# instadeepai/FrameDiPT

Measured on AMD Instinct MI355X. Metric: residue*diffusion-steps/sec, higher is better.
Workload: dtype fp16

## Files before the change

framedipt_amd/csrc/frames.hip:

```cpp
#include "common.hpp"
#include "kernels.hpp"
#include "philox.hpp"

#pragma clang fp contract(off)

__device__ __forceinline__ void d_quat_to_rot(const float* q, float* R) {
  const float a = q[0], b = q[1], c = q[2], d = q[3];
  R[0] = a * a + b * b - c * c - d * d; R[1] = 2 * b * c - 2 * a * d; R[2] = 2 * b * d + 2 * a * c;
  R[3] = 2 * b * c + 2 * a * d; R[4] = a * a - b * b + c * c - d * d; R[5] = 2 * c * d - 2 * a * b;
  R[6] = 2 * b * d - 2 * a * c; R[7] = 2 * c * d + 2 * a * b; R[8] = a * a - b * b - c * c + d * d;
}
__device__ __forceinline__ void d_quat_mul(const float* p, const float* q, float* o) {
  o[0] = p[0] * q[0] - p[1] * q[1] - p[2] * q[2] - p[3] * q[3];
  o[1] = p[0] * q[1] + p[1] * q[0] + p[2] * q[3] - p[3] * q[2];
  o[2] = p[0] * q[2] - p[1] * q[3] + p[2] * q[0] + p[3] * q[1];
  o[3] = p[0] * q[3] + p[1] * q[2] - p[2] * q[1] + p[3] * q[0];
}
__device__ __forceinline__ void d_quat_mul_vec(const float* q, const float* v, float* o) {
  o[0] = -q[1] * v[0] - q[2] * v[1] - q[3] * v[2];
  o[1] = q[0] * v[0] + q[2] * v[2] - q[3] * v[1];
  o[2] = q[0] * v[1] - q[1] * v[2] + q[3] * v[0];
  o[3] = q[0] * v[2] + q[1] * v[1] - q[2] * v[0];
}
__device__ __forceinline__ void d_invert_quat(const float* q, float* o) {
// ... 573 lines not shown
int fd_split_rigids(long n, const float* t7, float cs, const float* res_mask, const float* fixed_mask, float* quat,
                    float* trans, float* dmask, FdStep step, hipStream_t st) {
  hipLaunchKernelGGL(split_rigids_kernel, dim3(cdiv(n, 256)), dim3(256), 0, st, n, t7, cs, res_mask, fixed_mask, quat, trans, dmask, step);
  FD_CHECK_LAUNCH();
  return FDIPT_OK;
}

__global__ void finish_kernel(long n, const float* __restrict__ quat, const float* __restrict__ trans, float cs,
                              const float* __restrict__ psi_un, int ld_psi, const float* __restrict__ gt_psi,
                              const float* __restrict__ fixed_mask, float* __restrict__ rigids,
                              float* __restrict__ psi) {
  const long r = (long)blockIdx.x * blockDim.x + threadIdx.x;
  if (r >= n) return;
  for (int c = 0; c < 4; ++c) rigids[r * 7 + c] = quat[r * 4 + c];
  for (int c = 0; c < 3; ++c) fd_st(rigids + r * 7 + 4 + c, trans[r * 3 + c] / cs);
  const float a = psi_un[r * ld_psi], bq = psi_un[r * ld_psi + 1];
  const float den = sqrtf(fmaxf(a * a + bq * bq, 1e-8f));
  const float dm = 1.f - fixed_mask[r];
  psi[r * 2] = dm * (a / den) + (1.f - dm) * gt_psi[r * 2];
  psi[r * 2 + 1] = dm * (bq / den) + (1.f - dm) * gt_psi[r * 2 + 1];
}
int fd_finish(long n, const float* quat, const float* trans, float cs, const float* psi_un, int ld_psi,
              const float* gt_psi, const float* fixed_mask, float* rigids, float* psi, hipStream_t st) {
  hipLaunchKernelGGL(finish_kernel, dim3(cdiv(n, 256)), dim3(256), 0, st, n, quat, trans, cs, psi_un, ld_psi, gt_psi,
                     fixed_mask, rigids, psi);
  FD_CHECK_LAUNCH();
  return FDIPT_OK;
}

struct FeatsExtra {
  const float *t7, *res_mask; float cs; float *quat, *trans, *dmask;
  const float *w1i, *w1j, *b1; int cz; float *pi, *pj;
  FdStep step;
};
template <bool KEPT>
__global__ void build_feats_kernel(int B, int N, int use_aatype, int E, const int32_t* __restrict__ aatype,
                                   const float* __restrict__ t_emb_, const float* __restrict__ t_emb_eps,
                                   const float* __restrict__ fixed_mask, const float* __restrict__ idx_emb,
                                   float* __restrict__ node_feat, int ld_node, float* __restrict__ pte, int ld_pte,
                                   FeatsExtra x) {
  __shared__ float pte_s[128];
  const FdStepRows at = fd_step_rows<KEPT>(x.step);
  const float* __restrict__ t_emb = t_emb_ + at.step * B * E;
  if (x.t7) x.t7 += at.state_in * B * N * 7;
  const long r = blockIdx.x;
  const int b = (int)(r / N);
  const float fm = fixed_mask[r];
  const int d1 = E + 1 + (use_aatype ? 21 : 0);
  if (x.t7 && threadIdx.x < 8) {
    const int c = threadIdx.x;
    if (c < 4) x.quat[r * 4 + c] = x.t7[r * 7 + c];
    else if (c < 7) x.trans[r * 3 + c - 4] = x.t7[r * 7 + c] * x.cs;
    else x.dmask[r] = (1.f - fm) * x.res_mask[r];
  }
  for (int c = threadIdx.x; c < ld_node; c += blockDim.x) {
    float v = 0.f;
    int cc = c;
    if (use_aatype) {
      if (c < 21) { v = (aatype[r] == c) ? 1.f : 0.f; cc = -1; } else cc = c - 21;
    }
    if (cc >= 0) {
      if (cc < E) v = (use_aatype && fm != 0.f) ? t_emb_eps[cc] : t_emb[b * E + cc];
      else if (cc == E) v = fm;
      else if (cc < 2 * E + 1) v = idx_emb[r * E + (cc - E - 1)];
    }
    node_feat[r * ld_node + c] = v;
    if (c < ld_pte) {
      pte[r * ld_pte + c] = c < d1 ? v : 0.f;
      if (x.pi && c < 128) pte_s[c] = c < d1 ? v : 0.f;
    }
  }
  if (!x.pi) return;
  __syncthreads();
  for (int c = threadIdx.x; c < x.cz; c += blockDim.x) {
    const float4* wi = (const float4*)(x.w1i + (long)c * ld_pte);
    const float4* wj = (const float4*)(x.w1j + (long)c * ld_pte);
    float si = 0.f, sj = 0.f;
    for (int k = 0; k < ld_pte / 4; ++k) {
      const float4 a = wi[k], bq = wj[k];
      const float p0 = pte_s[4 * k], p1 = pte_s[4 * k + 1], p2 = pte_s[4 * k + 2], p3 = pte_s[4 * k + 3];
      si = fmaf(p3, a.w, fmaf(p2, a.z, fmaf(p1, a.y, fmaf(p0, a.x, si))));
      sj = fmaf(p3, bq.w, fmaf(p2, bq.z, fmaf(p1, bq.y, fmaf(p0, bq.x, sj))));
    }
    x.pi[r * x.cz + c] = si + x.b1[c];
    x.pj[r * x.cz + c] = sj;
  }
}
int fd_build_feats(int B, int N, int use_aatype, int E, const int32_t* aatype, const float* t_emb, const float* t_emb_eps,
                   const float* fixed_mask, const float* idx_emb, float* node_feat, int ld_node, float* pte, int ld_pte,
                   const float* t7, const float* res_mask, float cs, float* quat, float* trans, float* dmask, const float* w1i,
                   const float* w1j, const float* b1, int cz, float* pi, float* pj, FdStep step, hipStream_t st) {
  if (use_aatype && (!aatype || !t_emb_eps)) return FDIPT_EINVAL;
  if (pi && (ld_pte > 128 || (ld_pte & 3))) return FDIPT_EINVAL;
  FeatsExtra x = {t7, res_mask, cs, quat, trans, dmask, w1i, w1j, b1, cz, pi, pj, step};
  const auto kernel = step.kept() ? build_feats_kernel<true> : build_feats_kernel<false>;
  hipLaunchKernelGGL(kernel, dim3(B * N), dim3(128), 0, st, B, N, use_aatype, E, aatype, t_emb, t_emb_eps,
                     fixed_mask, idx_emb, node_feat, ld_node, pte, ld_pte, x);
  FD_CHECK_LAUNCH();
  return FDIPT_OK;
}

int fd_rot_score(int B, int N, const float* qt, int ld_t, const float* q0, int ld_0, const double* sigma,
                 const float* res_mask, double* score, hipStream_t st) {
  ScoreTail x = {};
  hipLaunchKernelGGL(rot_score_kernel<false>, dim3(cdiv((long)B * N, FD_THREADS / RS_LANES)), dim3(FD_THREADS), 0, st, B, N, qt, ld_t, q0,
                     ld_0, sigma, res_mask, score, x);
  FD_CHECK_LAUNCH();
  return FDIPT_OK;
}
int fd_score_tail(int B, int N, const float* rigids_t, const float* quat, const float* trans, float cs, const float* psi_un,
                  int ld_psi, const float* gt_psi, const float* fixed_mask, const float* res_mask, const double* sigma,
                  const float* t, float min_b, float max_b, float* rigids, float* psi, double* rot_score, float* trans_score,
                  float* ca_out, const float* hid, int ld_hid, int c_hid, const float* torf_w, const float* torf_b,
                  const double* score_table, const double* omega_edges, int n_omega, const int32_t* aatype, const void* bb_tables,
                  float* atom37, float* atom14, FdStep step, hipStream_t st) {
  if (hid && ((c_hid & 3) || (ld_hid & 3))) return FDIPT_EINVAL;
  if (score_table && (!omega_edges || n_omega < 2)) return FDIPT_EINVAL;
  if ((atom37 || atom14) && !bb_tables) return FDIPT_EINVAL;
  ScoreTail x = {trans, cs, psi_un, ld_psi, gt_psi, fixed_mask, t, min_b, max_b, rigids, psi, trans_score, ca_out,
                 hid, torf_w, torf_b, ld_hid, c_hid, score_table, omega_edges, n_omega, aatype, (const BackboneTables*)bb_tables, atom37, atom14,
                 step};
  const auto kernel = step.kept() ? rot_score_kernel<true> : rot_score_kernel<false>;
  hipLaunchKernelGGL(kernel, dim3(cdiv((long)B * N, FD_THREADS / RS_LANES)), dim3(FD_THREADS), 0, st, B, N, rigids_t, 7,
                     quat, 4, sigma, res_mask, rot_score, x);
  FD_CHECK_LAUNCH();
  return FDIPT_OK;
}
int fd_trans_score(int B, int N, const float* tt, int ld_t, const float* t0, int ld_0, const float* t, float min_b,
                   float max_b, float cs, const float* res_mask, float* score, hipStream_t st) {
// ... 592 lines not shown
```

framedipt_amd/csrc/kernels.hpp:

```cpp
#pragma once
#include <hip/hip_runtime.h>
#include <stdint.h>

typedef unsigned short half_t;

struct EdgeTransArgs {
  int B, N;
  const void* z_in;
  void* z_out;
  const float* e;
  const void *w1, *w2, *wf;
  const float *b1, *b2, *bf, *gamma, *beta;
  const float* res_mask;
  float* trace;
  unsigned long long* clock = nullptr;
};

struct EdgeEmbedArgs {
  int B, N, n_rel, rel_off, num_bins;
  const float* pi;
  const float* pj;
  const float* rtab;
  const float* dtab;
  const float* edges;
// ... 301 lines not shown
                 const float* beta, const float* rowmask, float* out, int ldo, hipStream_t st);
int fd_f32_to_half(long n, const float* in, half_t* out, hipStream_t st);
int fd_edge_transition(int precision, int cz, int cb, const EdgeTransArgs& a, hipStream_t st);
int fd_edge_embed(int precision, int cz, const EdgeEmbedArgs& a, hipStream_t st);
int fd_attention(int precision, int ipa, const AttnArgs& a, hipStream_t st);
int fd_ipa_attention_f32_supported(const AttnArgs& a);
int fd_ipa_attention_f32(const AttnArgs& a, hipStream_t st);
int fd_opair(int precision, const OPairArgs& a, hipStream_t st, int long_keys = 0);
int fd_opair_mfma_eligible(int precision, const OPairArgs& a, int long_keys = 0);
int fd_opair_pz(const OPairArgs& a, hipStream_t st);
int fd_pair_bias2(int B, int N, int H, const void* z, const void* wb, const float* bb, float* out, int frag, hipStream_t st);
int fd_pair_bias_f32(long n_pairs, int H, int CZ, const float* z, const float* wb, const float* bb, float* out, hipStream_t st);
int fd_points(const PointsArgs& a, hipStream_t st);
int fd_compose_q_update(long n, float* quat, float* trans, const float* upd, int ld_upd, const float* mask, hipStream_t st);
struct FdStep {
  const int32_t* cursor = nullptr;
  const int32_t* frame_rows = nullptr;
  int ring = 0;
  bool valid() const { return (ring & ~1) == 0 && (cursor || (!frame_rows && !ring)); }
  bool kept() const { return frame_rows != nullptr || ring != 0; }
};
struct FdStepRows { long step, state_in, state_out, frame; };
template <bool KEPT = true>
__device__ __forceinline__ FdStepRows fd_step_rows(const FdStep& s) {
  if (!s.cursor) return {0, 0, 0, 0};
  const long k = s.cursor[0];
  if (!KEPT) return {k, k, k + 1, k};
  return {k, s.ring ? (k & 1) : k, s.ring ? ((k + 1) & 1) : k + 1, s.frame_rows ? (long)s.frame_rows[k] : k};
}
int fd_split_rigids(long n, const float* t7, float cs, const float* res_mask, const float* fixed_mask, float* quat,
                    float* trans, float* dmask, FdStep step, hipStream_t st);
int fd_finish(long n, const float* quat, const float* trans, float cs, const float* psi_un, int ld_psi,
              const float* gt_psi, const float* fixed_mask, float* rigids, float* psi, hipStream_t st);
int fd_build_feats(int B, int N, int use_aatype, int E, const int32_t* aatype, const float* t_emb, const float* t_emb_eps,
                   const float* fixed_mask, const float* idx_emb, float* node_feat, int ld_node, float* pte, int ld_pte,
                   const float* t7, const float* res_mask, float cs, float* quat, float* trans, float* dmask, const float* w1i,
                   const float* w1j, const float* b1, int cz, float* pi, float* pj, FdStep step, hipStream_t st);
int fd_score_tail(int B, int N, const float* rigids_t, const float* quat, const float* trans, float cs, const float* psi_un,
                  int ld_psi, const float* gt_psi, const float* fixed_mask, const float* res_mask, const double* sigma,
                  const float* t, float min_b, float max_b, float* rigids, float* psi, double* rot_score, float* trans_score,
                  float* ca_out, const float* hid, int ld_hid, int c_hid, const float* torf_w, const float* torf_b,
                  const double* score_table, const double* omega_edges, int n_omega, const int32_t* aatype, const void* bb_tables,
                  float* atom37, float* atom14, FdStep step, hipStream_t st);
int fd_rot_score(int B, int N, const float* qt, int ld_t, const float* q0, int ld_0, const double* sigma,
                 const float* res_mask, double* score, hipStream_t st);
int fd_trans_score(int B, int N, const float* tt, int ld_t, const float* t0, int ld_0, const float* t, float min_b,
                   float max_b, float cs, const float* res_mask, float* score, hipStream_t st);
int fd_backbone(int n, const float* t7, const float* rot, const float* trans, int ld_trans, const float* psi,
                const int32_t* aatype, const void* tables, float* atom37, float* atom14, hipStream_t st,
                FdStep step = {});
```

framedipt_amd/csrc/model.hip:

```cpp
#include <math.h>
#include <string.h>

#include <vector>

#include "common.hpp"
#include "kernels.hpp"

struct LinW { long w, b; int out, in; };
struct LNW { long g, b; int d; };
#define FD_MAX_BLOCKS 8
#define FD_MAX_TL 4
struct TfLayer { LinW inp, outp, l1, l2; LNW n1, n2; };
struct BlockW {
  long head_w;
  LinW q, kv, qp, kvp, lb, dz, out, rbf;
  LNW ipa_ln;
  LinW skip;
  TfLayer tf[FD_MAX_TL];
  LinW post, t1, t2, t3;
  LNW tln;
  LinW bb;
  LinW et_init, et1, et2, etf;
  LNW et_ln;
};
// ... 560 lines not shown
}

enum { OP_ALL, OP_EMBED, OP_POINTS, OP_IPA, OP_ET };
struct OpSel {
  int kind = OP_ALL, block = 0;
  const float* node_in = nullptr;
  const void* z_in = nullptr;
  void* z_out = nullptr;
  float* node_out = nullptr;
  float* out = nullptr;
  float *qp = nullptr, *kp = nullptr, *vp = nullptr;
};

enum NodeForm { NF_GEMM, NF_ROWBLOCK, NF_ROWS16 };
enum SkipAt { SKIP_PER_BLOCK, SKIP_EMBED16, SKIP_SPLITK };
enum OutProj { OUT_GEMM, OUT_DEDICATED, OUT_SPLITK_SPLIT };
enum NodeRows { NR_PROJ, NR_POINTS, NR_LAUNCH };
enum SeqAttn { SEQ_FUSED, SEQ_BF16, SEQ_F32, SEQ_GENERIC };
enum PostAt { POST_TAIL, POST_CHAIN, POST_GEMM };
enum EtKind { ET_GEMM, ET_CHAIN, ET_ET3, ET_ET4 };
enum EtRows { ETR_IMAGES, ETR_ROWS, ETR_FOLDED };
struct ForwardPlan {
  int op;
  bool bf, fused_node;
  NodeForm embed, tail, transition, torsion;
  SkipAt skip;
  OutProj outproj;
  int slices;
  bool feats_fused, ee_bias, et_bias, pz;
  bool ee_table;
  bool stream;
  bool a3, probs_h16;
  bool vpt, proj2, merged, proj_pts, vt_lo, init_fused;
  NodeRows node_rows;
  SeqAttn seq;
  PostAt post;
  bool et_widths;
  EtKind et;
  EtRows et_rows;
  bool torf_fused, bb_fold;
  bool regpair;
  bool ipa_bias_f32, ipa_attn_f32;
  bool x;
  bool refused;
};
static const char kImage = 0;

static ForwardPlan plan_forward(const FdiptDims* d, const Inventory& iv, const DLayout& L, int B, int N, int op, int n_rel, bool trace_edge,
                                bool pair_embed) {
  const unsigned f = (unsigned)d->kernel_flags;
  const bool generic_attn = f & FDIPT_KF_GENERIC_ATTN, unfolded = f & FDIPT_KF_UNFOLDED;
  const int cs = d->c_s, cz = d->c_z, H = d->no_heads, C = d->c_hidden, Pq = d->no_qk_points, Pv = d->no_v_points;
  const int Np = (N + 31) / 32 * 32;
  ForwardPlan p = {};
  p.op = op;
  p.bf = half_mode(d);
  p.fused_node = use_chain(d);
  const bool rows16 = p.fused_node && !(f & FDIPT_KF_ROWS32) && N <= 512;
  p.embed = p.fused_node && (L.kn_pad == 72 || L.kn_pad == 88) ? (rows16 ? NF_ROWS16 : NF_ROWBLOCK) : NF_GEMM;
  p.torsion = p.tail = p.transition = p.fused_node ? (rows16 ? NF_ROWS16 : NF_ROWBLOCK) : NF_GEMM;
  const bool splitk = p.fused_node && iv.feat_dim >= 1024;
  if (!splitk || unfolded || op != OP_ALL) p.skip = SKIP_PER_BLOCK;
  else if (p.embed == NF_ROWS16 && skip16_image(d)) p.skip = SKIP_EMBED16;
  else p.skip = SKIP_SPLITK;
  p.feats_fused = L.d1_pad <= 128 && (L.d1_pad & 3) == 0 && !unfolded && op == OP_ALL;
  Attn3Args a3 = {};
  a3.B = B; a3.N = N; a3.H = H; a3.Np = Np; a3.vpt = (const half_t*)&kImage;
  OPairArgs oa = {};
  oa.B = B; oa.N = N; oa.H = H; oa.CZ = cz; oa.CD = cz / 4; oa.wdz_img = p.bf && dz_images(d) ? &kImage : nullptr;
  p.stream = (f & FDIPT_KF_STREAM_ATTN) && p.bf && !generic_attn && N <= 2048;
  const int n_attn = p.stream ? 2048 : 1024;
  const bool opair_mfma = fd_opair_mfma_eligible(op_precision(d), oa, p.stream);
  p.a3 = p.bf && cz == 128 && C == 256 && Pq == 8 && Pv == 12 && !generic_attn &&
         (p.stream ? fd_attention3_stream_supported(a3) : fd_attention3_supported(a3));
  p.probs_h16 = p.a3 && opair_mfma && 2 * Np <= 4 * N;
  const bool bias_rule = bias_images(d) && C == 256 && Pq == 8 && Pv == 12 && N <= n_attn && !generic_attn && !unfolded;
  p.regpair = use_regpair(d);
  p.ee_bias = bias_rule && p.regpair;
  p.et_bias = bias_rule;
  p.et_widths = iv.cb == 128 && iv.hid == 384 && cz == 128;
  const bool reg_ok = p.fused_node && p.et_widths && p.regpair;
  if (reg_ok && !(f & FDIPT_KF_ET3) && fd_edge_transition4_supported(N)) p.et = ET_ET4;
  else if (reg_ok && fd_edge_transition3_supported(N)) p.et = ET_ET3;
  else p.et = p.fused_node ? ET_CHAIN : ET_GEMM;
  p.et_rows = unfolded ? ETR_ROWS : p.et == ET_ET4 && p.transition == NF_ROWS16 && op == OP_ALL ? ETR_FOLDED : ETR_IMAGES;
  p.pz = op == OP_ALL && p.probs_h16 && p.et == ET_ET4 && bias_rule && !(f & FDIPT_KF_PASS_Z);
  {
    EdgeEmbedArgs ep = {};
    ep.B = B; ep.N = N; ep.n_rel = n_rel; ep.num_bins = d->num_bins; ep.H = H;
    p.ee_table = ee_table_static(d, B, N) && op == OP_ALL && p.ee_bias && p.pz && !trace_edge && !pair_embed && n_rel > 0 && n_rel <= ee_table_max_rel(N) &&
                 ee_table_rows_ok(B, N, n_rel, d->num_bins) && fd_edge_embed2_table_supported(ep);
  }
  p.vpt = p.a3 && Pv == 12;
  ProjArgs pj = {};
  pj.B = B; pj.N = N; pj.H = H; pj.C = C; pj.K = cs; pj.PT = iv.proj_out - 3 * H * C; pj.Np = Np; pj.lda = cs;
  pj.W_img = proj_image(d) ? &kImage : nullptr;
  pj.W_img_lo = pj.W_img && p.fused_node ? &kImage : nullptr;
  p.merged = p.a3 && pj.W_img_lo && merged_image(d) && !(f & FDIPT_KF_NO_MERGE) && op == OP_ALL && fd_ipa_proj2_supported(pj);
  pj.merged = p.merged;
  p.proj_pts = p.merged && !(f & FDIPT_KF_POINTS_LAUNCH) && p.vpt && points_image(d) && fd_ipa_proj2_points_supported(pj, Pq, Pv);
  if (p.proj_pts) pj.PT = fd_ipa_proj2_points_cols(H, C) - H * C;
  p.proj2 = p.a3 && fd_ipa_proj2_supported(pj);
  p.vt_lo = p.merged || (p.proj2 && pj.W_img_lo);
  p.node_rows = !p.merged || p.proj_pts ? NR_PROJ : p.vpt && (H & 1) == 0 && cs == 256 ? NR_POINTS : NR_LAUNCH;
  const int th = d->tfmr_heads, hd = iv.d_t / th;
  const bool seq_ok = p.stream ? fd_seq_attention_stream_supported(N, th, hd) : fd_seq_attention_supported(N, th, hd);
  if (p.fused_node && !generic_attn && seq_ok && fd_seq_qkv_supported(N, th, iv.d_t)) p.seq = SEQ_FUSED;
  else if (p.bf && !generic_attn && seq_ok) p.seq = SEQ_BF16;
  else if (!p.bf && !generic_attn && fd_seq_attention_f32_supported(N, th, hd, 3 * iv.d_t)) p.seq = SEQ_F32;
  else p.seq = SEQ_GENERIC;
  p.ipa_bias_f32 = !p.bf && H == 8 && cz == 128;
  p.ipa_attn_f32 = !p.bf && !generic_attn;
  p.init_fused = p.proj2 && p.seq == SEQ_FUSED && !unfolded;
  if (!splitk) p.outproj = OUT_GEMM;
  else p.outproj = p.merged && outproj_image(d, iv) ? OUT_DEDICATED : OUT_SPLITK_SPLIT;
  p.slices = p.outproj == OUT_DEDICATED ? fd_outproj_split_slices() : 3;
  p.post = !p.fused_node ? POST_GEMM : unfolded ? POST_CHAIN : POST_TAIL;
  p.torf_fused = (cs & 3) == 0 && !unfolded;
  p.bb_fold = !unfolded;
  p.x = d->precision == FDIPT_PREC_F16X;
  const unsigned x_refused = FDIPT_KF_ET3 | FDIPT_KF_GENERIC_PAIR | FDIPT_KF_GENERIC_ATTN | FDIPT_KF_UNFUSED_NODE | FDIPT_KF_STREAM_ATTN;
  const bool runs_et = op == OP_ALL || op == OP_ET;
  p.refused = p.x && ((f & x_refused) || (runs_et && p.et != ET_ET4) || !p.fused_node || N > 1024);
  return p;
}

enum WarmOf { WARM_QKV, WARM_TAIL, WARM_POST, WARM_TRANSITION, WARM_TRANSITION32, WARM_ET_ROWS, WARM_ET_FOLDED, WARM_TORSION };
struct Fwd {
  const FdiptDims* d;
  const Inventory& iv;
  const DLayout& L;
  const WS& w;
  const ForwardPlan& p;
  const float* P;
  const char* D;
  char* W;
  const void* setup;
  const FdiptForwardArgs* a;
  hipStream_t st;
  int B, N, R, Np;
  size_t NN;
  const float* res_mask = a->res_mask;
  float* F(size_t off) const { return (float*)(W + off); }
  FdStep step() const { return FdStep{a->step_cursor, a->frame_rows, a->state_ring}; }
  const void* WM(const LinW& l) const { return p.bf ? (const void*)((const half_t*)(D + L.h16_base) + l.w) : (const void*)(P + l.w); }
  int lin(const LinW& l, const float* A, int lda, const float* res, int ldr, const float* rm, int relu, float* out, int ldo) const {
// ... 18 lines not shown
    const DBlock& db = L.blk[b];
    const int cs = d->c_s, dt = iv.d_t;
    const unsigned tb = (unsigned)fd_chain_image_bytes(cs, cs);
    switch (next) {
      case WARM_QKV: {
        const unsigned n = (unsigned)fd_chain_image_bytes(3 * dt, dt);
        return L2Warm{{D + db.ch.inp[l], D + db.lo.inp[l], nullptr}, {n, n, 0}};
      }
      case WARM_TAIL: {
        if (p.tail == NF_ROWS16) return L2Warm{{D + db.lo.o16[l][0], D + db.lo.o16[l][1], nullptr}, {db.lo.tail16_run[l], db.lo.tail16_run[l], 0}};
        const unsigned wimg = (unsigned)fd_chain_image_bytes(dt, dt);
        return L2Warm{{D + db.ch.outp[l], D + db.ch.l1[l], D + db.ch.l2[l]}, {wimg, wimg, wimg}};
      }
      case WARM_POST: return L2Warm{{D + db.ch.post, nullptr, nullptr}, {(unsigned)fd_chain_image_bytes(cs, dt), 0, 0}};
      case WARM_TRANSITION:
        if (p.transition == NF_ROWS16) return L2Warm{{D + db.lo.tr16[0][0], D + db.lo.tr16[0][1], nullptr}, {db.lo.tr16_run, db.lo.tr16_run, 0}};
        return L2Warm{{D + db.ch.t1, D + db.ch.t2, D + db.lo.t1}, {tb, db.ch.t23_run, db.lo.t_run}};
      case WARM_TRANSITION32:
        return L2Warm{{D + db.ch.t1, D + db.ch.t2, D + db.ch.t3}, {tb, tb, tb}};
      case WARM_ET_ROWS: {
        const unsigned ei = (unsigned)fd_chain_image_bytes(iv.cb, cs), r4 = (unsigned)fd_chain_image_bytes(2 * (iv.hid + d->c_z), iv.cb);
        return L2Warm{{D + db.ch.et_init, D + db.ch.r4w, D + db.lo.et_init}, {ei, r4, db.lo.et_run}};
      }
      case WARM_ET_FOLDED:
        return L2Warm{{D + db.lo.ei16[0], D + db.lo.ei16[1], nullptr}, {db.lo.et16_run, db.lo.et16_run, 0}};
      case WARM_TORSION:
        if (p.torsion == NF_ROWS16) return L2Warm{{D + L.tor16[0][0], D + L.tor16[0][1], nullptr}, {L.tor16_run, L.tor16_run, 0}};
        return L2Warm{{D + L.ch_tor1, D + L.ch_tor2, D + L.lo_tor1}, {tb, tb, L.lo_tor_run}};
    }
    return L2Warm{};
  }
  int embed_stage() const {
    const int cs = d->c_s, cz = d->c_z;
    RC(fd_build_feats(B, N, d->use_aatype, d->index_embed, a->aatype, a->t_emb, a->t_emb_eps, a->fixed_mask, a->idx_emb, F(w.node_feat),
                      L.kn_pad, F(w.pte), L.d1_pad, p.feats_fused ? a->rigids_t : nullptr, a->res_mask, d->coordinate_scaling, F(w.quat),
                      F(w.trans), F(w.dmask), (const float*)(D + L.w1i), (const float*)(D + L.w1j), (const float*)(D + L.b1), cz,
                      p.feats_fused ? F(w.pi) : nullptr, F(w.pj), step(), st));
    if (p.embed == NF_GEMM) {
      RC(fd_linear(op_precision(d), R, cs, L.kn_pad, F(w.node_feat), L.kn_pad, D + L.ne0_pad, L.kn_pad, P + iv.ne0.b, nullptr, 0, nullptr, 1,
                   F(w.h_a), cs, st));
      RC(lin(iv.ne2, F(w.h_a), cs, nullptr, 0, nullptr, 1, F(w.h_b), cs));
      RC(lin(iv.ne4, F(w.h_b), cs, nullptr, 0, nullptr, 0, F(w.h_a), cs));
      RC(fd_layernorm(R, cs, F(w.h_a), cs, nullptr, 0, P + iv.neln.g, P + iv.neln.b, a->res_mask, F(w.node0), cs, st));
    } else {
      const bool r16 = p.embed == NF_ROWS16;
      RowBlockArgs r;
      r.M = R; r.in = F(w.node_feat); r.ld_in = L.kn_pad;
      r.w0 = D + (r16 ? L.ne16[0][0] : L.ch_ne0); r.w1 = D + (r16 ? L.ne16[1][0] : L.ch_ne2); r.w2 = D + (r16 ? L.ne16[2][0] : L.ch_ne4);
      r.w0l = D + (r16 ? L.ne16[0][1] : L.lo_ne0); r.w1l = D + (r16 ? L.ne16[1][1] : L.lo_ne2); r.w2l = D + (r16 ? L.ne16[2][1] : L.lo_ne4);
      r.b0 = P + iv.ne0.b; r.b1 = P + iv.ne2.b; r.b2 = P + iv.ne4.b;
      r.gamma = P + iv.neln.g; r.beta = P + iv.neln.b; r.rowmask_post = a->res_mask; r.out = F(w.node0); r.ld_out = cs;
      if (p.skip == SKIP_EMBED16) {
        r.w3 = D + L.skip16[0]; r.w3l = D + L.skip16[1]; r.b3 = (const float*)(D + L.skip_b);
        r.out2 = F(w.skip_all); r.ld_out2 = d->num_blocks * d->c_skip;
        r.warm = L2Warm{{r.w0, r.w0l, r.w3}, {L.ne16_run, L.ne16_run, L.skip16_run}};
      }
      if (r16) RC(fd_node_embed16(r, L.kn_pad, st));
      else RC(fd_rowblock(L.kn_pad == 72 ? FD_RB_NODE_EMBED_72 : FD_RB_NODE_EMBED_88, r, st));
    }
    if (!p.feats_fused) {
      RC(fd_linear(FDIPT_PREC_F32, R, cz, L.d1_pad, F(w.pte), L.d1_pad, D + L.w1i, L.d1_pad, (const float*)(D + L.b1), nullptr, 0,
                   nullptr, 0, F(w.pi), cz, st));
      RC(fd_linear(FDIPT_PREC_F32, R, cz, L.d1_pad, F(w.pte), L.d1_pad, D + L.w1j, L.d1_pad, nullptr, nullptr, 0, nullptr, 0,
                   F(w.pj), cz, st));
    }
    EdgeEmbedArgs ea;
    ea.B = B; ea.N = N; ea.n_rel = a->n_rel; ea.rel_off = a->rel_off; ea.num_bins = d->num_bins;
    ea.pi = F(w.pi); ea.pj = F(w.pj); ea.rtab = (const float*)setup; ea.dtab = d->num_bins > 0 ? (const float*)(D + L.dtab) : nullptr;
    ea.edges = d->num_bins > 0 ? (const float*)(D + L.edges) : nullptr; ea.seq_idx = a->seq_idx; ea.sc_ca = a->sc_ca_t;
    ea.w2 = WM(iv.ee2); ea.w3 = WM(iv.ee4); ea.b2 = P + iv.ee2.b; ea.b3 = P + iv.ee4.b;
    ea.gamma = P + iv.eeln.g; ea.beta = P + iv.eeln.b; ea.res_mask = a->res_mask; ea.z_out = W + w.z;
    ea.trace = a->trace_edge; ea.reserve_cus = a->reserve_cus;
    ea.wb_img = p.ee_bias ? D + L.blk[0].wb_img4 : nullptr; ea.bb = (const float*)(D + L.blk[0].bb); ea.bias_out = F(w.bias); ea.H = d->no_heads;
    if (p.pz) {
      ea.wdz_img = D + L.blk[0].wdz_imgp; ea.wdz_img_lo = D + L.blk[0].wdz_imgp_lo; ea.bdz = P + iv.blk[0].dz.b; ea.pz_out = (half_t*)(W + w.pz);
    }
    if (p.ee_table) {
      ea.fixed_mask = a->fixed_mask; ea.table = W + w.ee_tab; ea.row_idx = (int32_t*)(W + w.ee_idx); ea.leaders = (int32_t*)(W + w.ee_lead);
      ea.rel_lead = (const int32_t*)((const char*)setup + setup_rel_lead(d, B, a->n_rel));
      RC(fd_edge_embed2_leaders(ea, st));
      RC(fd_edge_embed2_table(ea, D + (p.x ? L.ee2x : L.ee2), st, p.x));
      ea.pz_out = nullptr;
      RC(fd_edge_embed2_spread(ea, st, 0));
    } else if (p.regpair) RC(fd_edge_embed2(ea, D + (p.x ? L.ee2x : L.ee2), st, p.x));
    else RC(fd_edge_embed(op_precision(d), cz, ea, st));
    return FDIPT_OK;
  }
  int ipa_project(int b, const float* node) const {
    const DBlock& db = L.blk[b];
    const int cs = d->c_s, H = d->no_heads, C = d->c_hidden, Pq = d->no_qk_points, Pv = d->no_v_points, PT = iv.proj_out - 3 * H * C;
    PointsArgs pa;
    pa.B = B; pa.N = N; pa.H = H; pa.Pq = Pq; pa.Pv = Pv; pa.quat = F(w.quat); pa.trans = F(w.trans);
    pa.qp = F(w.qp); pa.kp = F(w.kp); pa.vp = F(w.vp); pa.rot = F(w.rot);
    pa.vpt = p.vpt ? (unsigned short*)(W + w.vpt) : nullptr; pa.Np = Np;
    if (!p.a3) {
      RC(fd_linear(op_precision(d), R, iv.proj_out, cs, node, cs, D + db.wproj, cs, (const float*)(D + db.bproj), nullptr, 0,
                   nullptr, 0, F(w.proj), iv.proj_out, st));
      pa.proj = F(w.proj); pa.ld = iv.proj_out; pa.q_off = 3 * H * C; pa.kv_off = 3 * H * C + 3 * H * Pq;
      return fd_points(pa, st);
    }
    pa.kpf = (unsigned short*)(W + w.kpf); pa.gamma = (const float*)(D + db.gamma); pa.res_mask = a->res_mask;
    ProjArgs pj;
    pj.B = B; pj.N = N; pj.H = H; pj.C = C; pj.K = cs; pj.PT = PT; pj.Np = Np; pj.A = node; pj.lda = cs;
    pj.W = D + db.wproj; pj.bias = (const float*)(D + db.bproj); pj.qscale = sqrtf(1.0f / (3.0f * (float)C));
    pj.Qb = (half_t*)(W + w.qb); pj.Kb = (half_t*)(W + w.kb); pj.Vt = (half_t*)(W + w.vt); pj.pts = F(w.pts);
    pj.zero_pads = first_block(b);
    pj.W_img = proj_image(d) ? D + db.wproj_img : nullptr;
    pj.W_img_lo = pj.W_img && p.fused_node ? D + db.wproj_img_lo : nullptr;
    if (p.merged) { pj.merged = 1; pj.W_img = D + db.wproj2_img; pj.W_img_lo = D + db.wproj2_img_lo; pj.bias = (const float*)(D + db.bproj2); }
    if (p.proj_pts) {
      pj.pts_img = 1; pj.W_img = D + db.wproj2p_img; pj.W_img_lo = D + db.wproj2p_img_lo; pj.bias = (const float*)(D + db.bproj2p);
      pj.PT = fd_ipa_proj2_points_cols(H, C) - H * C;
      pj.quat = pa.quat; pj.trans = pa.trans; pj.gamma = pa.gamma; pj.res_mask = pa.res_mask; pj.rot = pa.rot; pj.qp = pa.qp;
// ... 274 lines not shown
                     a->res_mask, a->so3_sigma, a->t, d->r3_min_b, d->r3_max_b, a->rigids, a->psi, a->rot_score, a->trans_score,
                     a->ca_out, p.torf_fused ? F(w.h_b) : nullptr, cs, cs, P + iv.torf.w, P + iv.torf.b, a->so3_score_table,
                     a->so3_omega_edges, a->so3_num_omega, a->aatype, bb_fold ? a->bb_tables : nullptr, bb_fold ? a->atom37 : nullptr,
                     bb_fold ? a->atom14 : nullptr, step(), st));
    if (atoms && !bb_fold && (a->atom37 || !a->frame_rows))
      RC(fd_backbone(R, a->rigids, nullptr, nullptr, 0, a->psi, a->aatype, a->bb_tables, a->atom37, a->frame_rows ? nullptr : a->atom14, st, step()));
    return FDIPT_OK;
  }
};

static int forward_impl(const FdiptDims* d, const float* P, const void* derived, const void* setup,
                        const FdiptForwardArgs* a, void* workspace, size_t workspace_bytes, fdipt_stream_t stream, const OpSel& op) {
  if (!dims_ok(d) || !P || !derived || !a || !workspace) return FDIPT_EINVAL;
  if (a->B <= 0 || a->N <= 0 || !a->res_mask) return FDIPT_EINVAL;
  if (op.kind == OP_ALL || op.kind == OP_EMBED) {
    if (!setup || !a->fixed_mask || (!a->sc_ca_t && d->num_bins > 0) || !a->seq_idx || !a->idx_emb || !a->t_emb) return FDIPT_EINVAL;
    if (d->use_aatype && (!a->aatype || !a->t_emb_eps)) return FDIPT_EINVAL;
  }
  if (op.kind == OP_ALL && (!a->rigids_t || !a->gt_psi || !a->t || !a->so3_sigma || !a->psi || !a->rot_score || !a->trans_score ||
                            !a->rigids))
    return FDIPT_EINVAL;
  if ((op.kind == OP_POINTS || op.kind == OP_IPA) && !a->rigids_t) return FDIPT_EINVAL;
  if (!FdStep{a->step_cursor, a->frame_rows, a->state_ring}.valid()) return FDIPT_EINVAL;
  if (op.kind != OP_ALL && op.kind != OP_EMBED && (op.block < 0 || op.block >= d->num_blocks - (op.kind == OP_ET ? 1 : 0))) return FDIPT_EINVAL;
  Inventory iv;
  DLayout L;
  WS w;
  build_inventory(d, iv);
  blob_walk(d, iv, L);
  const int B = a->B, N = a->N, R = B * N;
  build_ws(d, iv, L, B, N, w);
  if (workspace_bytes < w.total) return FDIPT_ESIZE;
  if ((long)B * N * N > 2000000000L / 1) return FDIPT_ESIZE;
  const ForwardPlan p = plan_forward(d, iv, L, B, N, op.kind, a->n_rel, a->trace_edge != nullptr, a->pair_embed != 0);
  if (p.refused) return FDIPT_EINVAL;
  const Fwd f = {d, iv, L, w, p, P, (const char*)derived, (char*)workspace, setup, a, (hipStream_t)stream, B, N, R, (N + 31) / 32 * 32, (size_t)R * N};
  if (a->trace_inner && (p.fused_node || p.outproj != OUT_GEMM)) return FDIPT_EINVAL;
  const size_t node_bytes = (size_t)R * d->c_s * 4, z_bytes = f.NN * d->c_z * L.esz;
  if (op.kind == OP_ALL || op.kind == OP_EMBED) RC(f.embed_stage());
  if (op.kind == OP_EMBED) {
    if (op.node_out) RC(f.d2d(op.node_out, f.F(w.node0), node_bytes));
    if (op.z_out) RC(f.d2d(op.z_out, f.W + w.z, z_bytes));
    return FDIPT_OK;
  }
  if (a->trace_node && op.kind == OP_ALL) RC(f.d2d(a->trace_node, f.F(w.node0), node_bytes));
  if (!p.feats_fused && a->rigids_t)
    RC(fd_split_rigids(R, a->rigids_t, d->coordinate_scaling, a->res_mask, a->fixed_mask ? a->fixed_mask : a->res_mask, f.F(w.quat),
                       f.F(w.trans), f.F(w.dmask), f.step(), f.st));
  if (op.kind != OP_ALL) {
    if (!op.node_in) return FDIPT_EINVAL;
    RC(f.d2d(f.F(w.node), op.node_in, node_bytes));
    if (op.kind != OP_POINTS) {
      if (!op.z_in) return FDIPT_EINVAL;
      RC(f.d2d(f.W + w.z, op.z_in, z_bytes));
    }
    const int b = op.block;
    if (op.kind == OP_ET) {
      RC(f.edge_transition_stage(b, f.F(w.node)));
      if (!op.z_out) return FDIPT_EINVAL;
      return f.d2d(op.z_out, f.W + w.z, z_bytes);
    }
    RC(f.ipa_project(b, f.F(w.node)));
    if (op.kind == OP_POINTS) {
      if (!op.qp || !op.kp || !op.vp) return FDIPT_EINVAL;
      const size_t qk = (size_t)R * d->no_heads * d->no_qk_points * 3 * 4;
      RC(f.d2d(op.qp, f.F(w.qp), qk));
      RC(f.d2d(op.kp, f.F(w.kp), qk));
// ... 6 lines not shown
  }
  const int cs = d->c_s, nsk = d->num_blocks * d->c_skip;
  if (p.skip == SKIP_SPLITK)
    RC(fd_linear_splitk_split(R, nsk, cs, 1, f.F(w.node0), cs, (const float*)(f.D + L.skip_w32), cs, (const float*)(f.D + L.skip_b),
                              nullptr, f.F(w.skip_all), 0, nsk, f.st));
  const float* node = f.F(w.node0);
  for (int b = 0; b < d->num_blocks; ++b) {
    const float* x;
    RC(f.ipa_project(b, node));
    RC(f.ipa_attend(b));
    RC(f.ipa_out(b, node));
    RC(f.seq_stage(b, &x));
    RC(f.inner(b, 2, x, iv.d_t, iv.d_t));
    RC(f.transition_stage(b, x));
    node = f.F(w.node);
    if (b < d->num_blocks - 1) RC(f.edge_transition_stage(b, node));
    if (a->trace_node) RC(f.d2d(a->trace_node + (size_t)(b + 1) * R * cs, node, node_bytes));
  }
  return f.heads_stage(node);
}

extern "C" {

int64_t fdipt_embed_table_rows(const FdiptDims* d, int B, int N, int n_rel) {
  if (!dims_ok(d) || B <= 0 || N <= 0 || n_rel <= 0) return 0;
  Inventory iv;
  DLayout L;
  build_inventory(d, iv);
  blob_walk(d, iv, L);
  const ForwardPlan p = plan_forward(d, iv, L, B, N, OP_ALL, n_rel, false, false);
  return p.ee_table && !p.refused ? (int64_t)n_rel * (d->num_bins + 1) : 0;
}

int fdipt_embed_table_leaders(const FdiptDims* d, const void* workspace, int B, int N, int n_rel, int32_t* out_dev) {
  if (!workspace || !out_dev || fdipt_embed_table_rows(d, B, N, n_rel) <= 0) return FDIPT_EINVAL;
  Inventory iv;
  DLayout L;
  WS w;
  build_inventory(d, iv);
  blob_walk(d, iv, L);
  build_ws(d, iv, L, B, N, w);
  if (hipDeviceSynchronize() != hipSuccess) return FDIPT_ELAUNCH;
  return hipMemcpy(out_dev, (const char*)workspace + w.ee_lead, (size_t)B * 4, hipMemcpyDeviceToDevice) == hipSuccess ? FDIPT_OK : FDIPT_ELAUNCH;
}

int fdipt_score_forward(const FdiptDims* d, const float* P, const void* derived, const void* setup,
                        const FdiptForwardArgs* a, void* workspace, size_t workspace_bytes, fdipt_stream_t stream) {
  return forward_impl(d, P, derived, setup, a, workspace, workspace_bytes, stream, OpSel{});
}

int fdipt_edge_embed_fwd(const FdiptDims* d, const float* P, const void* derived, const void* setup, const FdiptForwardArgs* a,
                         float* node_out, void* z_out, void* workspace, size_t workspace_bytes, fdipt_stream_t stream) {
  OpSel op;
  op.kind = OP_EMBED; op.node_out = node_out; op.z_out = z_out;
  return forward_impl(d, P, derived, setup, a, workspace, workspace_bytes, stream, op);
}

static FdiptForwardArgs op_args(int B, int N, const float* rigids_t, const float* res_mask) {
  FdiptForwardArgs a;
  memset(&a, 0, sizeof(a));
  a.B = B; a.N = N; a.rigids_t = rigids_t; a.res_mask = res_mask;
  return a;
}
int fdipt_ipa_project_points(const FdiptDims* d, const float* P, const void* derived, int block, int B, int N, const float* node,
                             const float* rigids, const float* res_mask, float* q_pts, float* k_pts, float* v_pts,
                             void* workspace, size_t workspace_bytes, fdipt_stream_t stream) {
// ... 41 lines not shown
```

include/fdipt.h:

```cpp
#ifndef FDIPT_H
#define FDIPT_H

#include <stddef.h>
#include <stdint.h>

#ifdef __cplusplus
extern "C" {
#endif

#define FDIPT_OK 0
#define FDIPT_EINVAL (-1)
#define FDIPT_ELAUNCH (-2)
#define FDIPT_ESIZE (-3)

#define FDIPT_PREC_F32 0
#define FDIPT_PREC_BF16 1
#define FDIPT_PREC_F16 2
#define FDIPT_PREC_F16X 3

#define FDIPT_KF_ET3 1
#define FDIPT_KF_GENERIC_PAIR 2
#define FDIPT_KF_GENERIC_ATTN 4
#define FDIPT_KF_UNFUSED_NODE 8
#define FDIPT_KF_UNFOLDED 16
// ... 50 lines not shown
  const int32_t* aatype;
  const float* gt_psi;
  const float* t;
  const float* t_emb;
  const float* t_emb_eps;
  const double* so3_sigma;
  const void* bb_tables;
  float* psi;
  double* rot_score;
  float* trans_score;
  float* rigids;
  float* atom37;
  float* atom14;
  float* trace_node;
  float* trace_edge;
  float* trace_inner;
  void** ev_start;
  void** ev_stop;
  float* ca_out;
  int32_t reserve_cus;
  int32_t pair_embed;
  unsigned long long* clock_out;
  const double* so3_score_table;
  const double* so3_omega_edges;
  int32_t so3_num_omega;
  const int32_t* step_cursor;
  const int32_t* frame_rows;
  int32_t state_ring;
} FdiptForwardArgs;

size_t fdipt_forward_workspace_bytes(const FdiptDims* dims, int B, int N);
int64_t fdipt_embed_table_rows(const FdiptDims* dims, int B, int N, int n_rel);
int fdipt_embed_table_leaders(const FdiptDims* dims, const void* workspace, int B, int N, int n_rel, int32_t* out_dev);
int fdipt_score_forward(const FdiptDims* dims, const float* params_f32, const void* derived, const void* setup,
                        const FdiptForwardArgs* args, void* workspace, size_t workspace_bytes, fdipt_stream_t stream);

int fdipt_edge_embed_fwd(const FdiptDims* dims, const float* params_f32, const void* derived, const void* setup,
                         const FdiptForwardArgs* args, float* node_out, void* z_out, void* workspace, size_t workspace_bytes,
                         fdipt_stream_t stream);
int fdipt_ipa_project_points(const FdiptDims* dims, const float* params_f32, const void* derived, int block, int B, int N,
                             const float* node, const float* rigids, const float* res_mask, float* q_pts, float* k_pts,
                             float* v_pts, void* workspace, size_t workspace_bytes, fdipt_stream_t stream);
int fdipt_ipa_attention_fwd(const FdiptDims* dims, const float* params_f32, const void* derived, int block, int B, int N,
                            const float* node, const void* z, const float* rigids, const float* res_mask, float* out,
                            void* workspace, size_t workspace_bytes, fdipt_stream_t stream);
int fdipt_edge_transition_fwd(const FdiptDims* dims, const float* params_f32, const void* derived, int block, int B, int N,
                              const float* node, const float* res_mask, const void* z_in, void* z_out, void* workspace,
                              size_t workspace_bytes, fdipt_stream_t stream);

int fdipt_se3_reverse_step(int B, int N, const float* rigids_t, const double* rot_score, const float* trans_score,
                           const float* diffuse_mask , const double* z_rot, const double* z_trans,
                           double t, double dt, double noise_scale, int center, int diffuse_rot, int diffuse_trans,
                           double so3_min_sigma, double so3_max_sigma, double r3_min_b, double r3_max_b,
                           double coordinate_scaling, float* rigids_out , float* out_rot ,
                           fdipt_stream_t stream);
int fdipt_se3_reverse_step_atoms(int B, int N, const float* rigids_t, const double* rot_score, const float* trans_score,
                                 const float* diffuse_mask, const double* z_rot, const double* z_trans, double t, double dt,
                                 double noise_scale, int center, int diffuse_rot, int diffuse_trans, double so3_min_sigma,
                                 double so3_max_sigma, double r3_min_b, double r3_max_b, double coordinate_scaling,
                                 float* rigids_out, float* out_rot, const float* psi, const int32_t* aatype,
                                 const void* tables, float* atom37, fdipt_stream_t stream);

int fdipt_se3_reverse_step_traj(int B, int N, const float* rigids_t, const double* rot_score, const float* trans_score,
                                const float* diffuse_mask, const double* z_rot, const double* z_trans, double t, double dt,
                                double noise_scale, int center, int diffuse_rot, int diffuse_trans, double so3_min_sigma,
                                double so3_max_sigma, double r3_min_b, double r3_max_b, double coordinate_scaling,
// ... 365 lines not shown
```

Before: 1.262 million.

## Fold edge-embed leader election into build_feats kernel as extra rider blocks

Adds B extra blocks to the build_feats launch that compute, per batch element, which earlier batch element produces identical first-layer edge features, and write the leader index. The separate fd_edge_embed2_leaders launch is skipped when this path is active. The goal is to save one kernel launch and its serialization per step. In exchange, the rider blocks run redundant first-layer matvecs and several block-wide barriers, and they may lengthen the feats kernel's tail.

```diff
diff --git a/framedipt_amd/csrc/frames.hip b/framedipt_amd/csrc/frames.hip
--- a/framedipt_amd/csrc/frames.hip
+++ b/framedipt_amd/csrc/frames.hip
@@ -629,7 +629,130 @@
   const float *t7, *res_mask; float cs; float *quat, *trans, *dmask;
   const float *w1i, *w1j, *b1; int cz; float *pi, *pj;
   FdStep step;
+  int n_lead;
+  const int32_t* rel_lead; int32_t* leaders;
 };
+template <int G>
+__device__ __forceinline__ void feats_first_layer(const float* p, int ld_pte, const float* __restrict__ w1i, const float* __restrict__ w1j,
+                                                  int c, float (&si)[G], float (&sj)[G]) {
+  const float4* wi = (const float4*)(w1i + (long)c * ld_pte);
+  const float4* wj = (const float4*)(w1j + (long)c * ld_pte);
+#pragma unroll
+  for (int g = 0; g < G; ++g) si[g] = sj[g] = 0.f;
+  auto step = [&](int k) {
+    const float4 a = wi[k], bq = wj[k];
+#pragma unroll
+    for (int g = 0; g < G; ++g) {
+      const float* q = p + g * ld_pte + 4 * k;
+      const float p0 = q[0], p1 = q[1], p2 = q[2], p3 = q[3];
+      si[g] = fmaf(p3, a.w, fmaf(p2, a.z, fmaf(p1, a.y, fmaf(p0, a.x, si[g]))));
+      sj[g] = fmaf(p3, bq.w, fmaf(p2, bq.z, fmaf(p1, bq.y, fmaf(p0, bq.x, sj[g]))));
+    }
+  };
+  if (G == 1) {
+    for (int k = 0; k < ld_pte / 4; ++k) step(k);
+  } else {
+#pragma unroll 1
+    for (int k = 0; k < ld_pte / 4; ++k) step(k);
+  }
+}
+#define FL_G 2
+#define FL_INFO 112
+__device__ __forceinline__ void feats_leader_rider(int b, int N, int E, const float* __restrict__ t_emb, const float* __restrict__ fixed_mask,
+                                                   int ld_pte, const FeatsExtra& x, float* smem) {
+  const int tid = threadIdx.x, nth = blockDim.x;
+  int* rep = (int*)(smem + FL_INFO);
+  int* vote = rep + 4;
+  int* cand = rep + 5;
+  float* cfm = smem + FL_INFO + 8;
+  auto uni = [](int v) { return __builtin_amdgcn_readfirstlane(v); };
+  auto reps = [&](int s, int* out) {
+    if (tid < 2) out[tid] = N;
+    __syncthreads();
+    for (int k = tid; k < N; k += nth) atomicMin(&out[fixed_mask[(long)s * N + k] != 0.f ? 1 : 0], k);
+    __syncthreads();
+  };
+  auto all = [&](int pred) {
+    if (tid == 0) *vote = 1;
+    __syncthreads();
+    if (!pred) *vote = 0;
+    __syncthreads();
+    const int r = uni(*vote);
+    __syncthreads();
+    return r;
+  };
+  auto put = [&](int g, int s, float fm) {
+    for (int c = tid; c < ld_pte; c += nth) smem[g * ld_pte + c] = c < E ? t_emb[s * E + c] : c == E ? fm : 0.f;
+  };
+  const float b1 = x.b1[tid];
+  reps(b, rep);
+  const int r0 = uni(rep[0]), r1 = uni(rep[1]), rl = x.rel_lead[b];
+  const float f0 = r0 < N ? fixed_mask[(long)b * N + r0] : 0.f, f1 = r1 < N ? fixed_mask[(long)b * N + r1] : 0.f;
+  float oi[2] = {0.f, 0.f}, oj[2] = {0.f, 0.f};
+  float si[FL_G], sj[FL_G];
+  bool have_own = false;
+  int lead = b, c = 0;
+  while (c < b && lead == b) {
+    int n = 0;
+    while (c < b && n < FL_G) {
+      const int s = c++;
+      if (x.rel_lead[s] != rl) continue;
+      reps(s, rep + 2);
+      const int q0 = uni(rep[2]), q1 = uni(rep[3]);
+      __syncthreads();
+      if ((r0 < N && q0 == N) || (r1 < N && q1 == N)) continue;
+      if (tid == 0) {
+        cand[n] = s;
+        cfm[2 * n] = q0 < N ? fixed_mask[(long)s * N + q0] : 0.f;
+        cfm[2 * n + 1] = q1 < N ? fixed_mask[(long)s * N + q1] : 0.f;
+      }
+      ++n;
+    }
+    if (!n) break;
+    __syncthreads();
+    int first = n;
+    for (int g = 0; g < n && first == n; ++g) {
+      const int s = uni(cand[g]);
+      int same = 1;
+      for (int k = tid; k < E; k += nth) same &= __float_as_uint(t_emb[b * E + k]) == __float_as_uint(t_emb[s * E + k]);
+      if (r0 < N) same &= __float_as_uint(cfm[2 * g]) == __float_as_uint(f0);
+      if (r1 < N) same &= __float_as_uint(cfm[2 * g + 1]) == __float_as_uint(f1);
+      if (all(same)) first = g;
+    }
+    if (first > 0) {
+      if (!have_own) {
+        __syncthreads();
+        put(0, b, f0);
+        put(1, b, f1);
+        __syncthreads();
+        feats_first_layer<FL_G>(smem, ld_pte, x.w1i, x.w1j, tid, si, sj);
+        oi[0] = si[0] + b1; oj[0] = sj[0];
+        oi[1] = si[1] + b1; oj[1] = sj[1];
+        have_own = true;
+      }
+      int same[FL_G];
+#pragma unroll
+      for (int g = 0; g < FL_G; ++g) same[g] = 1;
+#pragma unroll
+      for (int cls = 0; cls < 2; ++cls) {
+        if ((cls ? r1 : r0) == N) continue;
+        __syncthreads();
+        for (int g = 0; g < FL_G; ++g) put(g, g < n ? uni(cand[g]) : b, g < n ? cfm[2 * g + cls] : 0.f);
+        __syncthreads();
+        feats_first_layer<FL_G>(smem, ld_pte, x.w1i, x.w1j, tid, si, sj);
+#pragma unroll
+        for (int g = 0; g < FL_G; ++g)
+          same[g] &= __float_as_uint(si[g] + b1) == __float_as_uint(oi[cls]) && __float_as_uint(sj[g]) == __float_as_uint(oj[cls]);
+      }
+#pragma unroll
+      for (int g = 0; g < FL_G; ++g)
+        if (g < first && g < n && lead == b && all(same[g])) lead = uni(cand[g]);
+    }
+    if (lead == b && first < n) lead = uni(cand[first]);
+    __syncthreads();
+  }
+  if (tid == 0) x.leaders[b] = lead;
+}
 template <bool KEPT>
 __global__ void build_feats_kernel(int B, int N, int use_aatype, int E, const int32_t* __restrict__ aatype,
                                    const float* __restrict__ t_emb_, const float* __restrict__ t_emb_eps,
@@ -639,8 +762,9 @@
   __shared__ float pte_s[128];
   const FdStepRows at = fd_step_rows<KEPT>(x.step);
   const float* __restrict__ t_emb = t_emb_ + at.step * B * E;
+  if (blockIdx.x < (unsigned)x.n_lead) return feats_leader_rider((int)blockIdx.x, N, E, t_emb, fixed_mask, ld_pte, x, pte_s);
   if (x.t7) x.t7 += at.state_in * B * N * 7;
-  const long r = blockIdx.x;
+  const long r = blockIdx.x - x.n_lead;
   const int b = (int)(r / N);
   const float fm = fixed_mask[r];
   const int d1 = E + 1 + (use_aatype ? 21 : 0);
@@ -670,28 +794,25 @@
   if (!x.pi) return;
   __syncthreads();
   for (int c = threadIdx.x; c < x.cz; c += blockDim.x) {
-    const float4* wi = (const float4*)(x.w1i + (long)c * ld_pte);
-    const float4* wj = (const float4*)(x.w1j + (long)c * ld_pte);
-    float si = 0.f, sj = 0.f;
-    for (int k = 0; k < ld_pte / 4; ++k) {
-      const float4 a = wi[k], bq = wj[k];
-      const float p0 = pte_s[4 * k], p1 = pte_s[4 * k + 1], p2 = pte_s[4 * k + 2], p3 = pte_s[4 * k + 3];
-      si = fmaf(p3, a.w, fmaf(p2, a.z, fmaf(p1, a.y, fmaf(p0, a.x, si))));
-      sj = fmaf(p3, bq.w, fmaf(p2, bq.z, fmaf(p1, bq.y, fmaf(p0, bq.x, sj))));
-    }
-    x.pi[r * x.cz + c] = si + x.b1[c];
-    x.pj[r * x.cz + c] = sj;
+    float si[1], sj[1];
+    feats_first_layer<1>(pte_s, ld_pte, x.w1i, x.w1j, c, si, sj);
+    x.pi[r * x.cz + c] = si[0] + x.b1[c];
+    x.pj[r * x.cz + c] = sj[0];
   }
 }
 int fd_build_feats(int B, int N, int use_aatype, int E, const int32_t* aatype, const float* t_emb, const float* t_emb_eps,
                    const float* fixed_mask, const float* idx_emb, float* node_feat, int ld_node, float* pte, int ld_pte,
                    const float* t7, const float* res_mask, float cs, float* quat, float* trans, float* dmask, const float* w1i,
-                   const float* w1j, const float* b1, int cz, float* pi, float* pj, FdStep step, hipStream_t st) {
+                   const float* w1j, const float* b1, int cz, float* pi, float* pj, FdStep step, hipStream_t st, const FeatsRiders& rd) {
   if (use_aatype && (!aatype || !t_emb_eps)) return FDIPT_EINVAL;
   if (pi && (ld_pte > 128 || (ld_pte & 3))) return FDIPT_EINVAL;
   FeatsExtra x = {t7, res_mask, cs, quat, trans, dmask, w1i, w1j, b1, cz, pi, pj, step};
+  if (rd.leaders) {
+    if (!rd.rel_lead || !pi || use_aatype || cz != 128 || FL_G * ld_pte > FL_INFO) return FDIPT_EINVAL;
+    x.n_lead = B; x.rel_lead = rd.rel_lead; x.leaders = rd.leaders;
+  }
   const auto kernel = step.kept() ? build_feats_kernel<true> : build_feats_kernel<false>;
-  hipLaunchKernelGGL(kernel, dim3(B * N), dim3(128), 0, st, B, N, use_aatype, E, aatype, t_emb, t_emb_eps,
+  hipLaunchKernelGGL(kernel, dim3(B * N + x.n_lead), dim3(128), 0, st, B, N, use_aatype, E, aatype, t_emb, t_emb_eps,
                      fixed_mask, idx_emb, node_feat, ld_node, pte, ld_pte, x);
   FD_CHECK_LAUNCH();
   return FDIPT_OK;
diff --git a/framedipt_amd/csrc/kernels.hpp b/framedipt_amd/csrc/kernels.hpp
--- a/framedipt_amd/csrc/kernels.hpp
+++ b/framedipt_amd/csrc/kernels.hpp
@@ -357,10 +357,15 @@
                     float* trans, float* dmask, FdStep step, hipStream_t st);
 int fd_finish(long n, const float* quat, const float* trans, float cs, const float* psi_un, int ld_psi,
               const float* gt_psi, const float* fixed_mask, float* rigids, float* psi, hipStream_t st);
+struct FeatsRiders {
+  const int32_t* rel_lead = nullptr;
+  int32_t* leaders = nullptr;
+};
 int fd_build_feats(int B, int N, int use_aatype, int E, const int32_t* aatype, const float* t_emb, const float* t_emb_eps,
                    const float* fixed_mask, const float* idx_emb, float* node_feat, int ld_node, float* pte, int ld_pte,
                    const float* t7, const float* res_mask, float cs, float* quat, float* trans, float* dmask, const float* w1i,
-                   const float* w1j, const float* b1, int cz, float* pi, float* pj, FdStep step, hipStream_t st);
+                   const float* w1j, const float* b1, int cz, float* pi, float* pj, FdStep step, hipStream_t st,
+                   const FeatsRiders& riders = FeatsRiders{});
 int fd_score_tail(int B, int N, const float* rigids_t, const float* quat, const float* trans, float cs, const float* psi_un,
                   int ld_psi, const float* gt_psi, const float* fixed_mask, const float* res_mask, const double* sigma,
                   const float* t, float min_b, float max_b, float* rigids, float* psi, double* rot_score, float* trans_score,
diff --git a/framedipt_amd/csrc/model.hip b/framedipt_amd/csrc/model.hip
--- a/framedipt_amd/csrc/model.hip
+++ b/framedipt_amd/csrc/model.hip
@@ -616,6 +616,7 @@
   bool stream;
   bool a3, probs_h16;
   bool vpt, proj2, merged, proj_pts, vt_lo, init_fused;
+  bool lead_rides;
   NodeRows node_rows;
   SeqAttn seq;
   PostAt post;
@@ -631,7 +632,7 @@
 static const char kImage = 0;
 
 static ForwardPlan plan_forward(const FdiptDims* d, const Inventory& iv, const DLayout& L, int B, int N, int op, int n_rel, bool trace_edge,
-                                bool pair_embed) {
+                                bool pair_embed, bool own_leaders = false) {
   const unsigned f = (unsigned)d->kernel_flags;
   const bool generic_attn = f & FDIPT_KF_GENERIC_ATTN, unfolded = f & FDIPT_KF_UNFOLDED;
   const int cs = d->c_s, cz = d->c_z, H = d->no_heads, C = d->c_hidden, Pq = d->no_qk_points, Pv = d->no_v_points;
@@ -696,6 +697,7 @@
   p.ipa_bias_f32 = !p.bf && H == 8 && cz == 128;
   p.ipa_attn_f32 = !p.bf && !generic_attn;
   p.init_fused = p.proj2 && p.seq == SEQ_FUSED && !unfolded;
+  p.lead_rides = p.ee_table && p.feats_fused && !d->use_aatype && cz == 128 && 2 * L.d1_pad <= 112 && !own_leaders;
   if (!splitk) p.outproj = OUT_GEMM;
   else p.outproj = p.merged && outproj_image(d, iv) ? OUT_DEDICATED : OUT_SPLITK_SPLIT;
   p.slices = p.outproj == OUT_DEDICATED ? fd_outproj_split_slices() : 3;
@@ -780,10 +782,15 @@
   }
   int embed_stage() const {
     const int cs = d->c_s, cz = d->c_z;
+    FeatsRiders riders;
+    if (p.lead_rides) {
+      riders.rel_lead = (const int32_t*)((const char*)setup + setup_rel_lead(d, B, a->n_rel));
+      riders.leaders = (int32_t*)(W + w.ee_lead);
+    }
     RC(fd_build_feats(B, N, d->use_aatype, d->index_embed, a->aatype, a->t_emb, a->t_emb_eps, a->fixed_mask, a->idx_emb, F(w.node_feat),
                       L.kn_pad, F(w.pte), L.d1_pad, p.feats_fused ? a->rigids_t : nullptr, a->res_mask, d->coordinate_scaling, F(w.quat),
                       F(w.trans), F(w.dmask), (const float*)(D + L.w1i), (const float*)(D + L.w1j), (const float*)(D + L.b1), cz,
-                      p.feats_fused ? F(w.pi) : nullptr, F(w.pj), step(), st));
+                      p.feats_fused ? F(w.pi) : nullptr, F(w.pj), step(), st, riders));
     if (p.embed == NF_GEMM) {
       RC(fd_linear(op_precision(d), R, cs, L.kn_pad, F(w.node_feat), L.kn_pad, D + L.ne0_pad, L.kn_pad, P + iv.ne0.b, nullptr, 0, nullptr, 1,
                    F(w.h_a), cs, st));
@@ -826,7 +833,7 @@
     if (p.ee_table) {
       ea.fixed_mask = a->fixed_mask; ea.table = W + w.ee_tab; ea.row_idx = (int32_t*)(W + w.ee_idx); ea.leaders = (int32_t*)(W + w.ee_lead);
       ea.rel_lead = (const int32_t*)((const char*)setup + setup_rel_lead(d, B, a->n_rel));
-      RC(fd_edge_embed2_leaders(ea, st));
+      if (!p.lead_rides) RC(fd_edge_embed2_leaders(ea, st));
       RC(fd_edge_embed2_table(ea, D + (p.x ? L.ee2x : L.ee2), st, p.x));
       ea.pz_out = nullptr;
       RC(fd_edge_embed2_spread(ea, st, 0));
@@ -1167,7 +1174,7 @@
   build_ws(d, iv, L, B, N, w);
   if (workspace_bytes < w.total) return FDIPT_ESIZE;
   if ((long)B * N * N > 2000000000L / 1) return FDIPT_ESIZE;
-  const ForwardPlan p = plan_forward(d, iv, L, B, N, op.kind, a->n_rel, a->trace_edge != nullptr, a->pair_embed != 0);
+  const ForwardPlan p = plan_forward(d, iv, L, B, N, op.kind, a->n_rel, a->trace_edge != nullptr, (a->pair_embed & 1) != 0, (a->pair_embed & 2) != 0);
   if (p.refused) return FDIPT_EINVAL;
   const Fwd f = {d, iv, L, w, p, P, (const char*)derived, (char*)workspace, setup, a, (hipStream_t)stream, B, N, R, (N + 31) / 32 * 32, (size_t)R * N};
   if (a->trace_inner && (p.fused_node || p.outproj != OUT_GEMM)) return FDIPT_EINVAL;
@@ -1240,6 +1247,16 @@
   return p.ee_table && !p.refused ? (int64_t)n_rel * (d->num_bins + 1) : 0;
 }
 
+int fdipt_embed_leaders_ride(const FdiptDims* d, int B, int N, int n_rel, int pair_embed) {
+  if (!dims_ok(d) || B <= 0 || N <= 0 || n_rel <= 0) return 0;
+  Inventory iv;
+  DLayout L;
+  build_inventory(d, iv);
+  blob_walk(d, iv, L);
+  const ForwardPlan p = plan_forward(d, iv, L, B, N, OP_ALL, n_rel, false, (pair_embed & 1) != 0, (pair_embed & 2) != 0);
+  return p.lead_rides && !p.refused ? 1 : 0;
+}
+
 int fdipt_embed_table_leaders(const FdiptDims* d, const void* workspace, int B, int N, int n_rel, int32_t* out_dev) {
   if (!workspace || !out_dev || fdipt_embed_table_rows(d, B, N, n_rel) <= 0) return FDIPT_EINVAL;
   Inventory iv;
diff --git a/include/fdipt.h b/include/fdipt.h
--- a/include/fdipt.h
+++ b/include/fdipt.h
@@ -106,6 +106,7 @@
 size_t fdipt_forward_workspace_bytes(const FdiptDims* dims, int B, int N);
 int64_t fdipt_embed_table_rows(const FdiptDims* dims, int B, int N, int n_rel);
 int fdipt_embed_table_leaders(const FdiptDims* dims, const void* workspace, int B, int N, int n_rel, int32_t* out_dev);
+int fdipt_embed_leaders_ride(const FdiptDims* dims, int B, int N, int n_rel, int pair_embed);
 int fdipt_score_forward(const FdiptDims* dims, const float* params_f32, const void* derived, const void* setup,
                         const FdiptForwardArgs* args, void* workspace, size_t workspace_bytes, fdipt_stream_t stream);
 
```

Measured after the change: 1.264 million (median of 6 runs). No clear change (+0.2%).
